# trzy/FasterRCNN

Measured on AMD Instinct MI355X. Metric: images/sec (600x1000) Faster-RCNN VGG-16 inference, higher is better.
Workload: dtype f32 (float32 tensors and accumulation; 15 GEMM layers in the f32x3 split-operand emulation = two fp16 terms per block-scaled operand, three fp16 MFMAs per product; 0 in f32x6 = three bf16 terms, six bf16 MFMAs; the other 2 on exact-f32 MFMA; strict exact-f32 everywhere: config.strict_f32_images_per_

## Files before the change

### fasterrcnn_amd/csrc/wino_x3f.hip

```cpp
#include "x3t.h"

namespace frcnn {

typedef _Float16 xf_f16x8 __attribute__((ext_vector_type(8)));

static constexpr int XF_TC = 16;
static constexpr int XF_HC = 2 * XF_TC + 2;
static constexpr int XF_PS = 20;
static constexpr int X3_HR = 10;


struct XfGeom { int tbx, tby, ncb, tw, th, xg; unsigned m_tbx, m_tby, m_ncb; int ntb; unsigned m_ntb; int g8; int n_items; };
__device__ __forceinline__ int xd_div(int n, int d, unsigned m) { return d == 1 ? n : (int)__umulhi((unsigned)n, m); }

typedef float xd_f32x2 __attribute__((ext_vector_type(2)));
typedef _Float16 xd_f16x2 __attribute__((ext_vector_type(2)));

static constexpr int XD_HP = XF_HC / 2;
static constexpr int XD_NDMA = 7;
static constexpr int XD_HBUF_BYTES = XD_NDMA * 256 * 16;
static constexpr int XD_HBUF_FLOATS = XD_HBUF_BYTES / 4;
typedef __attribute__((address_space(3))) void* xd_lds_ptr;
static constexpr int XD_MS = 68;
static constexpr int XD_M_BYTES = 16 * 32 * XD_MS * 4;
static constexpr int XD_SC_OFFSET = XD_M_BYTES;
static constexpr int XD_CM_OFFSET = XD_SC_OFFSET + 16 * 64 * 4 + 64 * 4;
static constexpr size_t XD_LDS_BYTES = XD_CM_OFFSET + 512 * 4;

template <int N> struct XdInt { static constexpr int value = N; };
#ifndef XD_ABLATE
#define XD_ABLATE 0
#endif

__device__ __forceinline__ float xd_rowmax16(float v)
{
    v = fmaxf(v, __builtin_bit_cast(float, __builtin_amdgcn_update_dpp(0, __builtin_bit_cast(int, v), 0x128, 0xf, 0xf, false)));
    v = fmaxf(v, __builtin_bit_cast(float, __builtin_amdgcn_update_dpp(0, __builtin_bit_cast(int, v), 0x124, 0xf, 0xf, false)));
    v = fmaxf(v, __builtin_bit_cast(float, __builtin_amdgcn_update_dpp(0, __builtin_bit_cast(int, v), 0x122, 0xf, 0xf, false)));
    v = fmaxf(v, __builtin_bit_cast(float, __builtin_amdgcn_update_dpp(0, __builtin_bit_cast(int, v), 0x121, 0xf, 0xf, false)));
    return v;
}

__device__ __forceinline__ f32x4 xd_sub4(f32x4 a, f32x4 b)
{
    xd_f32x2 a0 = {a[0], a[1]}, a1 = {a[2], a[3]}, b0 = {b[0], b[1]}, b1 = {b[2], b[3]}, r0, r1;
    asm("v_pk_add_f32 %0, %1, %2 neg_lo:[0,1] neg_hi:[0,1]" : "=v"(r0) : "v"(a0), "v"(b0));
    asm("v_pk_add_f32 %0, %1, %2 neg_lo:[0,1] neg_hi:[0,1]" : "=v"(r1) : "v"(a1), "v"(b1));
    return f32x4{r0[0], r0[1], r1[0], r1[1]};
}

__device__ __forceinline__ void xd_slot_tile(int s, int& ty, int& tx)
{
    ty = (int)((0xF00F0FF0u >> s) & 1u);
    tx = s - 4 * ((s + 4) >> 3);
}

__device__ __forceinline__ void xd_lds_barrier()
{
    asm volatile("s_waitcnt lgkmcnt(0)\n\ts_barrier" ::: "memory");
}


__device__ __forceinline__ bool xd_block_to_tile(const XfGeom& gm, int b, int& cb, int& bx, int& by, int& map)
{
    if (gm.xg == 2) {
        const int xcd = b & 7, s = b >> 3;
        if (gm.ncb >= 8) {
            const int k = xd_div(s, gm.ntb, gm.m_ntb);
            cb = xcd + 8 * k;
            b = s - k * gm.ntb;
        } else {
            const int g = gm.g8, sub = xd_div(xcd, gm.ncb, gm.m_ncb);
            cb = xcd - sub * gm.ncb;
            b = s * g + sub;
            if (b >= gm.ntb) return false;
        }
    } else if (gm.xg) {
        const int xcd = b & 7, q = b >> 3, qq = xd_div(q, gm.ncb, gm.m_ncb);
        cb = q - qq * gm.ncb;
        b = qq * 8 + xcd;
    } else {
        const int qq = xd_div(b, gm.ncb, gm.m_ncb);
        cb = b - qq * gm.ncb;
        b = qq;
    }
    const int b1 = xd_div(b, gm.tbx, gm.m_tbx);
    bx = b - b1 * gm.tbx;
    map = xd_div(b1, gm.tby, gm.m_tby);
    by = b1 - map * gm.tby;
    return true;
}


typedef unsigned xp_u32x4_t __attribute__((ext_vector_type(4)));


__device__ __forceinline__ float xd_rowmax16_scatter16(const float (&v)[16])
{
    float n0, n1, n2, n3, n4, n5, n6, n7;
    asm volatile("s_nop 1\n\t"
        "v_max_f32_dpp %0, %8, %8 row_ror:8 row_mask:0xf bank_mask:0x3\n\tv_max_f32_dpp %1, %9, %9 row_ror:8 row_mask:0xf bank_mask:0x3\n\t"
        "v_max_f32_dpp %2, %10, %10 row_ror:8 row_mask:0xf bank_mask:0x3\n\tv_max_f32_dpp %3, %11, %11 row_ror:8 row_mask:0xf bank_mask:0x3\n\t"
        "v_max_f32_dpp %4, %12, %12 row_ror:8 row_mask:0xf bank_mask:0x3\n\tv_max_f32_dpp %5, %13, %13 row_ror:8 row_mask:0xf bank_mask:0x3\n\t"
        "v_max_f32_dpp %6, %14, %14 row_ror:8 row_mask:0xf bank_mask:0x3\n\tv_max_f32_dpp %7, %15, %15 row_ror:8 row_mask:0xf bank_mask:0x3\n\t"
        "v_max_f32_dpp %0, %16, %16 row_ror:8 row_mask:0xf bank_mask:0xc\n\tv_max_f32_dpp %1, %17, %17 row_ror:8 row_mask:0xf bank_mask:0xc\n\t"
        "v_max_f32_dpp %2, %18, %18 row_ror:8 row_mask:0xf bank_mask:0xc\n\tv_max_f32_dpp %3, %19, %19 row_ror:8 row_mask:0xf bank_mask:0xc\n\t"
        "v_max_f32_dpp %4, %20, %20 row_ror:8 row_mask:0xf bank_mask:0xc\n\tv_max_f32_dpp %5, %21, %21 row_ror:8 row_mask:0xf bank_mask:0xc\n\t"
        "v_max_f32_dpp %6, %22, %22 row_ror:8 row_mask:0xf bank_mask:0xc\n\tv_max_f32_dpp %7, %23, %23 row_ror:8 row_mask:0xf bank_mask:0xc"
        : "=&v"(n0), "=&v"(n1), "=&v"(n2), "=&v"(n3), "=&v"(n4), "=&v"(n5), "=&v"(n6), "=&v"(n7)
        : "v"(v[0]), "v"(v[1]), "v"(v[2]), "v"(v[3]), "v"(v[4]), "v"(v[5]), "v"(v[6]), "v"(v[7]),
          "v"(v[8]), "v"(v[9]), "v"(v[10]), "v"(v[11]), "v"(v[12]), "v"(v[13]), "v"(v[14]), "v"(v[15]));
    float m0, m1, m2, m3;
    asm volatile(
        "v_max_f32_dpp %0, %4, %4 row_ror:12 row_mask:0xf bank_mask:0x5\n\tv_max_f32_dpp %1, %5, %5 row_ror:12 row_mask:0xf bank_mask:0x5\n\t"
        "v_max_f32_dpp %2, %6, %6 row_ror:12 row_mask:0xf bank_mask:0x5\n\tv_max_f32_dpp %3, %7, %7 row_ror:12 row_mask:0xf bank_mask:0x5\n\t"
        "v_max_f32_dpp %0, %8, %8 row_ror:4 row_mask:0xf bank_mask:0xa\n\tv_max_f32_dpp %1, %9, %9 row_ror:4 row_mask:0xf bank_mask:0xa\n\t"
        "v_max_f32_dpp %2, %10, %10 row_ror:4 row_mask:0xf bank_mask:0xa\n\tv_max_f32_dpp %3, %11, %11 row_ror:4 row_mask:0xf bank_mask:0xa\n\t"
        "v_max_f32_dpp %0, %0, %0 quad_perm:[2,3,0,1] row_mask:0xf bank_mask:0xf\n\tv_max_f32_dpp %1, %1, %1 quad_perm:[2,3,0,1] row_mask:0xf bank_mask:0xf\n\t"
        "v_max_f32_dpp %2, %2, %2 quad_perm:[2,3,0,1] row_mask:0xf bank_mask:0xf\n\tv_max_f32_dpp %3, %3, %3 quad_perm:[2,3,0,1] row_mask:0xf bank_mask:0xf\n\t"
        "v_max_f32_dpp %0, %0, %0 quad_perm:[1,0,3,2] row_mask:0xf bank_mask:0xf\n\tv_max_f32_dpp %1, %1, %1 quad_perm:[1,0,3,2] row_mask:0xf bank_mask:0xf\n\t"
        "v_max_f32_dpp %2, %2, %2 quad_perm:[1,0,3,2] row_mask:0xf bank_mask:0xf\n\tv_max_f32_dpp %3, %3, %3 quad_perm:[1,0,3,2] row_mask:0xf bank_mask:0xf\n\t"
        "s_nop 1"
        : "=&v"(m0), "=&v"(m1), "=&v"(m2), "=&v"(m3)
        : "v"(n0), "v"(n1), "v"(n2), "v"(n3), "v"(n4), "v"(n5), "v"(n6), "v"(n7));
    const int q = (int)(threadIdx.x & 3);
    return q == 0 ? m0 : q == 1 ? m1 : q == 2 ? m2 : m3;
}
__device__ __forceinline__ float xd_rowmax16_scatter4(const float (&v)[4])
{
    float n0, n1, m;
    asm volatile("s_nop 1\n\t"
        "v_max_f32_dpp %0, %3, %3 row_ror:8 row_mask:0xf bank_mask:0x3\n\tv_max_f32_dpp %1, %4, %4 row_ror:8 row_mask:0xf bank_mask:0x3\n\t"
        "v_max_f32_dpp %0, %5, %5 row_ror:8 row_mask:0xf bank_mask:0xc\n\tv_max_f32_dpp %1, %6, %6 row_ror:8 row_mask:0xf bank_mask:0xc\n\t"
        "s_nop 1\n\t"
        "v_max_f32_dpp %2, %0, %0 row_ror:12 row_mask:0xf bank_mask:0x5\n\tv_max_f32_dpp %2, %1, %1 row_ror:4 row_mask:0xf bank_mask:0xa\n\t"
        "s_nop 1\n\t"
        "v_max_f32_dpp %2, %2, %2 quad_perm:[2,3,0,1] row_mask:0xf bank_mask:0xf\n\t"
        "s_nop 1\n\t"
        "v_max_f32_dpp %2, %2, %2 quad_perm:[1,0,3,2] row_mask:0xf bank_mask:0xf\n\t"
        "s_nop 1"
        : "=&v"(n0), "=&v"(n1), "=&v"(m)
        : "v"(v[0]), "v"(v[1]), "v"(v[2]), "v"(v[3]));
    return m;
}

#ifndef XD_EARLY_HALO
#define XD_EARLY_HALO 1
#endif
static constexpr int XD_FIRST = 1, XD_EARLY = XD_EARLY_HALO ? 2 : 0, XD_LAST = 4;

template <bool POOL, bool TWO>
__global__ __launch_bounds__(256, 1)
void wino_x3d_kernel(const float* __restrict__ x_maps, const float* __restrict__ cmax_maps, const unsigned char* __restrict__ ublob,
                     const float* __restrict__ bias, float* __restrict__ y_maps, int H, int W, int Cin, int Cout, int u_rbt, int relu,
                     XfGeom gm, float* __restrict__ cmax_out_maps)
{
#ifdef XD_CLOCKS
    const unsigned long long xd_t_in = __builtin_amdgcn_s_memrealtime();
#endif
    extern __shared__ __attribute__((aligned(16))) unsigned char smem_xf[];
    float* const hbuf0 = reinterpret_cast<float*>(smem_xf);

#ifndef XD_PERSIST
    const int tid = threadIdx.x, lane = tid & 63;
    const int wave = __builtin_amdgcn_readfirstlane(tid >> 6);
#endif
    const int K16 = Cin >> 4;

#ifdef XD_PERSIST
    for (int item = blockIdx.x; item < gm.n_items; item += gridDim.x) {
    int tid_l = threadIdx.x;
#if XD_PERSIST >= 2
    asm volatile("" : "+v"(tid_l));
#endif
    const int tid = tid_l, lane = tid & 63;
    const int wave = __builtin_amdgcn_readfirstlane((int)threadIdx.x >> 6);
#else
    {
    const int item = blockIdx.x;
#endif
    int cb, bx, by, map;
    if (!xd_block_to_tile(gm, item, cb, bx, by, map)) {
#ifdef XD_PERSIST
        continue;
#else
        return;
#endif
    }
    const float* __restrict__ const x = x_maps + (size_t)map * H * W * Cin;
    const float* __restrict__ const cmax = cmax_maps + (size_t)map * H * W;
    float* __restrict__ const y = y_maps + (size_t)map * (POOL ? (size_t)(H >> 1) * (W >> 1) : (size_t)H * W) * Cout;
    float* __restrict__ const cmax_out = cmax_out_maps ? cmax_out_maps + (size_t)map * (POOL ? (size_t)(H >> 1) * (W >> 1) : (size_t)H * W) : nullptr;

    const __amdgpu_buffer_rsrc_t xrs = __builtin_amdgcn_make_buffer_rsrc(const_cast<float*>(x), 0, H * W * Cin * (int)sizeof(float), 0x00020000);
    const __amdgpu_buffer_rsrc_t mrs = __builtin_amdgcn_make_buffer_rsrc(const_cast<float*>(cmax), 0, H * W * (int)sizeof(float), 0x00020000);

    const int tl = lane & 31, kh = lane >> 5;
    int tyl, txl;
    xd_slot_tile(tl, tyl, txl);
    float mult[2], vinv[2];

    const int hy0 = 8 * by - 1, hx0 = 2 * XF_TC * bx - 1;
    const int wave_u = __builtin_amdgcn_readfirstlane(wave);
    int h_src[XD_NDMA];
    auto halo_source = [&](auto IT) {
        constexpr int it = decltype(IT)::value;
        const unsigned P = (unsigned)((it * 4 + wave) * 64 + lane);
        const unsigned slot = __umul24(P, 52429u) >> 18, part = P - 5u * slot;
        const unsigned hr = __umul24(slot, 1928u) >> 16, rem = slot - (unsigned)XF_HC * hr;
        const unsigned par = rem >= (unsigned)XD_HP ? 1u : 0u, hc = 2u * (rem - par * (unsigned)XD_HP) + par;
        const int gy = hy0 + (int)hr, gx = hx0 + (int)hc;
        bool inb = (part < 4u) & ((unsigned)gy < (unsigned)H) & ((unsigned)gx < (unsigned)W);
        if (it == XD_NDMA - 1) inb &= hr < (unsigned)X3_HR;
        const unsigned off = (__umul24((unsigned)gy, (unsigned)W) + (unsigned)gx) * (unsigned)(Cin * 4) + 16u * part;
        h_src[it] = inb ? (int)off : (int)0xFFFFFFF0u;
    };
    __amdgpu_buffer_rsrc_t xrs_ring = xrs;
    auto dma_halo = [&](float* hb, int chunk_off, auto IT0, auto IT1, const __amdgpu_buffer_rsrc_t& rs) {
        if (XD_ABLATE & 8) return;
#pragma unroll
        for (int it = decltype(IT0)::value; it < decltype(IT1)::value; ++it)
            __builtin_amdgcn_raw_ptr_buffer_load_lds(rs, (xd_lds_ptr)(reinterpret_cast<unsigned char*>(hb) + (it * 4 + wave_u) * 1024), 16, h_src[it],
                                                     chunk_off, 0, 0);
    };

    xf_f16x8 U[2][4][2][2];
    const __amdgpu_buffer_rsrc_t urs = __builtin_amdgcn_make_buffer_rsrc(const_cast<unsigned char*>(ublob), 0, 16 * K16 * u_rbt * HX_RB, 0x00020000);
    const int chunk_stride = u_rbt * HX_RB;
    int ubase[4];
#pragma unroll
    for (int j = 0; j < 4; ++j) ubase[j] = ((4 * wave + j) * K16 * u_rbt + 2 * cb) * HX_RB;
    const int lane16 = lane * 16;
    auto load_u = [&](int chunk, auto SET, auto J) {
        constexpr int set = decltype(SET)::value, j = decltype(J)::value;
        const int so = ubase[j] + chunk * chunk_stride;
#pragma unroll
        for (int ct = 0; ct < 2; ++ct)
#pragma unroll
            for (int t = 0; t < 2; ++t)
                U[set][j][ct][t] = __builtin_bit_cast(xf_f16x8, __builtin_amdgcn_raw_buffer_load_b128(urs, lane16, so + ct * HX_RB + t * HX_PIECE, 0));
    };

    f32x16 acc[2][4][2];

    const int a1 = wave == 0 ? 0 : (wave == 2 ? 2 : 1);
    const int a2 = wave == 0 ? 2 : (wave == 2 ? 1 : (wave == 1 ? 2 : 3));
    const float rsgn = wave != 1 ? -1.0f : 1.0f;
    const int d_lane = (4 * tyl * XD_HP + txl) * XF_PS + 8 * kh;
    float r[4][8];
    f32x4 du0, du1, dw0, dw1;
    auto read_d = [&](const float* hb, int h, int bb) {
        const float* p1 = hb + d_lane + (((4 * h + a1) * 2 + (bb & 1)) * XD_HP + (bb >> 1)) * XF_PS;
        const float* p2 = hb + d_lane + (((4 * h + a2) * 2 + (bb & 1)) * XD_HP + (bb >> 1)) * XF_PS;
        du0 = *reinterpret_cast<const f32x4*>(p1); du1 = *reinterpret_cast<const f32x4*>(p1 + 4);
        dw0 = *reinterpret_cast<const f32x4*>(p2); dw1 = *reinterpret_cast<const f32x4*>(p2 + 4);
    };
    auto read_d_lo = [&](const float* hb, int h, int bb) {
        const float* p1 = hb + d_lane + (((4 * h + a1) * 2 + (bb & 1)) * XD_HP + (bb >> 1)) * XF_PS;
        const float* p2 = hb + d_lane + (((4 * h + a2) * 2 + (bb & 1)) * XD_HP + (bb >> 1)) * XF_PS;
        du0 = *reinterpret_cast<const f32x4*>(p1);
        dw0 = *reinterpret_cast<const f32x4*>(p2);
    };
    auto read_d_hi = [&](const float* hb, int h, int bb) {
        const float* p1 = hb + d_lane + (((4 * h + a1) * 2 + (bb & 1)) * XD_HP + (bb >> 1)) * XF_PS;
        const float* p2 = hb + d_lane + (((4 * h + a2) * 2 + (bb & 1)) * XD_HP + (bb >> 1)) * XF_PS;
        du1 = *reinterpret_cast<const f32x4*>(p1 + 4);
        dw1 = *reinterpret_cast<const f32x4*>(p2 + 4);
    };
    auto make_r = [&](int bb, int half, int hs) {
        const bool scaled = bb == 1 || bb == 2;
#pragma unroll
        for (int e = 0; e < 4; ++e) {
            float v = half == 0 ? __builtin_fmaf(dw0[e], rsgn, du0[e]) : __builtin_fmaf(dw1[e], rsgn, du1[e]);
            if (scaled) asm volatile("v_mul_f32 %0, %1, %2" : "=v"(v) : "v"(v), "v"(mult[hs]));
            r[bb][4 * half + e] = v;
        }
    };
    unsigned vhi[2][4], vlo[2][4];
    float tt[4];
    auto v_adds = [&](int h, int j, int e2) {
#pragma unroll
        for (int q = 0; q < 4; ++q) {
            const int e = 2 * e2 + q;
            tt[q] = j == 0 ? __builtin_fmaf(r[0][e], mult[h], -r[2][e]) : j == 1 ? r[1][e] + r[2][e] : j == 2 ? r[2][e] - r[1][e]
                                                                                                   : __builtin_fmaf(r[3][e], -mult[h], r[1][e]);
        }
    };
    auto v_hi = [&](int slot, int e2) {
        unsigned ha, hb;
        asm("v_cvt_pk_f16_f32 %0, %1, %2" : "=v"(ha) : "v"(tt[0]), "v"(tt[1]));
        asm("v_cvt_pk_f16_f32 %0, %1, %2" : "=v"(hb) : "v"(tt[2]), "v"(tt[3]));
        vhi[slot][e2] = ha;
        vhi[slot][e2 + 1] = hb;
    };
    auto v_lo = [&](int slot, int e2) {
        unsigned la, lb;
        asm("v_fma_mixlo_f16 %0, %2, 1.0, -%6 op_sel:[0,0,0] op_sel_hi:[0,0,1]\n\tv_fma_mixlo_f16 %1, %4, 1.0, -%7 op_sel:[0,0,0] op_sel_hi:[0,0,1]\n\t"
            "v_fma_mixhi_f16 %0, %3, 1.0, -%6 op_sel:[0,0,1] op_sel_hi:[0,0,1]\n\tv_fma_mixhi_f16 %1, %5, 1.0, -%7 op_sel:[0,0,1] op_sel_hi:[0,0,1]"
            : "=&v"(la), "=&v"(lb) : "v"(tt[0]), "v"(tt[1]), "v"(tt[2]), "v"(tt[3]), "v"(vhi[slot][e2]), "v"(vhi[slot][e2 + 1]));
        vlo[slot][e2] = la;
        vlo[slot][e2 + 1] = lb;
    };
    auto frag = [&](const unsigned (&q)[4]) { return __builtin_bit_cast(xf_f16x8, uint4{q[0], q[1], q[2], q[3]}); };
#define XD_MFMA(SET, H_, J_, CT, UT, VV) \
    do { if (!(XD_ABLATE & 16)) acc[H_][J_][CT] = __builtin_amdgcn_mfma_f32_32x32x16_f16(U[SET][J_][CT][UT], VV, acc[H_][J_][CT], 0, 0, 0); } while (0)
#define XD_MFMA0(SET, H_, J_, CT, UT, VV) \
    do { if (first) acc[H_][J_][CT] = __builtin_amdgcn_mfma_f32_32x32x16_f16(U[SET][J_][CT][UT], VV, xd_zero16, 0, 0, 0); else XD_MFMA(SET, H_, J_, CT, UT, VV); } while (0)
#define XD_FENCE() __builtin_amdgcn_sched_barrier(0)
#define XD_IF(BIT, STMT) do { if (!(XD_ABLATE & (BIT))) { STMT; } } while (0)

#ifdef XD_STEPS
    unsigned long long xd_step_acc[8] = {0, 0, 0, 0, 0, 0, 0, 0}, xd_step_last = 0;
#endif
    auto step = [&](int ucb, int hso, int hso_next, float* hcur, float* hnxt, float* hthird_, auto PAR, auto S, auto FLAGS) {
        constexpr int par = decltype(PAR)::value, s = decltype(S)::value;
#ifdef XD_STEPS
        {
            const unsigned long long now = __builtin_readcyclecounter();
            if (xd_step_last != 0) xd_step_acc[(s + 7) & 7] += now - xd_step_last;
            xd_step_last = now;
        }
#endif
        constexpr bool first = (decltype(FLAGS)::value & XD_FIRST) != 0, early = (decltype(FLAGS)::value & XD_EARLY) != 0,
                       last = (decltype(FLAGS)::value & XD_LAST) != 0;
        const f32x16 xd_zero16 = {};
        constexpr int h = s >> 2, j = s & 3, slot = s & 1, nslot = slot ^ 1;
        constexpr int nh = s == 3 ? 1 : s == 7 ? 0 : h, nj = (j + 1) & 3;
        constexpr int rb = j == 0 ? 0 : j == 1 ? 2 : j == 2 ? 1 : 3;
        constexpr int prb = j == 0 ? 3 : j == 1 ? 0 : j == 2 ? 2 : 1;
        constexpr int rh = h ^ 1;
        constexpr int prh = j == 0 ? h : rh;
        constexpr bool col = !(last && h == 1), pcol = !(last && s >= 5), form = !(last && s == 7);
        const float* rsrc = h == 0 ? hcur : hnxt;
        const xf_f16x8 vh = frag(vhi[slot]), vl = frag(vlo[slot]);
        XD_MFMA0(par, h, j, 0, 1, vh);
        if (col) XD_IF(2, read_d_lo(rsrc, rh, rb));
        if (form) XD_IF(1, v_adds(nh, nj, 0));
        XD_FENCE();
        XD_MFMA0(par, h, j, 1, 1, vh);
        if (form) XD_IF(1, v_hi(nslot, 0));
        if (pcol) XD_IF(2, make_r(prb, 1, prh));
        XD_FENCE();
        XD_MFMA(par, h, j, 0, 0, vh);
        if (form) XD_IF(1, v_lo(nslot, 0));
        if (col) XD_IF(2, read_d_hi(rsrc, rh, rb));
        if (s == 4 && !last) dma_halo(hcur, hso, XdInt<0>{}, XdInt<4>{}, xrs_ring);
        if (early && !last && !(XD_EARLY_HALO == 2 && TWO) && s == 0) dma_halo(XD_EARLY_HALO == 2 ? hthird_ : hnxt, hso_next + (XD_EARLY_HALO == 2 ? 64 : 0), XdInt<0>{}, XdInt<4>{}, xrs);
        if (early && !last && !(XD_EARLY_HALO == 2 && TWO) && s == 1) dma_halo(XD_EARLY_HALO == 2 ? hthird_ : hnxt, hso_next + (XD_EARLY_HALO == 2 ? 64 : 0), XdInt<4>{}, XdInt<XD_NDMA>{}, xrs);
        XD_FENCE();
        XD_MFMA(par, h, j, 1, 0, vh);
        if (form) XD_IF(1, v_adds(nh, nj, 2));
        if (form) XD_IF(1, v_hi(nslot, 2));
        XD_FENCE();
        XD_MFMA(par, h, j, 0, 0, vl);
        if (form) XD_IF(1, v_lo(nslot, 2));
        if (!last && !(XD_ABLATE & 4)) {
            const int so = ubase[s >> 1] + ucb;
            U[par ^ 1][s >> 1][s & 1][0] = __builtin_bit_cast(xf_f16x8, __builtin_amdgcn_raw_buffer_load_b128(urs, lane16 + (s & 1) * HX_RB, so, 0));
            U[par ^ 1][s >> 1][s & 1][1] = __builtin_bit_cast(xf_f16x8, __builtin_amdgcn_raw_buffer_load_b128(urs, lane16 + (s & 1) * HX_RB + HX_PIECE, so, 0));
        }
        XD_FENCE();
        XD_MFMA(par, h, j, 1, 0, vl);
        if (col) XD_IF(2, make_r(rb, 0, rh));
        if (s == 3) {
            if (early) asm volatile("s_waitcnt vmcnt(%0)" ::"n"(XD_EARLY_HALO == 2 ? (last ? 0 : TWO ? 8 : 15) : (last ? 0 : 6)) : "memory");
            else asm volatile("s_waitcnt vmcnt(15)" ::: "memory");
            xd_lds_barrier();
        }
        if (s == 5 && !last) dma_halo(hcur, hso, XdInt<4>{}, XdInt<XD_NDMA>{}, xrs_ring);
        XD_FENCE();
    };
    float *hcur = hbuf0, *hnxt = hbuf0 + XD_HBUF_FLOATS, *hthird = hbuf0 + 2 * XD_HBUF_FLOATS;
    auto chunk = [&](int c, auto PAR, auto FLAGS) {
        const int ucb = (c + 1) * chunk_stride, hso = (c + 3 < K16 ? c + 3 : K16 - 1) * 64, hson = (c + 1) * 64;
        xrs_ring = __builtin_amdgcn_make_buffer_rsrc(const_cast<float*>(x), 0, c + 3 < K16 ? H * W * Cin * (int)sizeof(float) : 0, 0x00020000);
        step(ucb, hso, hson, hcur, hnxt, hthird, PAR, XdInt<0>{}, FLAGS); step(ucb, hso, hson, hcur, hnxt, hthird, PAR, XdInt<1>{}, FLAGS);
        step(ucb, hso, hson, hcur, hnxt, hthird, PAR, XdInt<2>{}, FLAGS); step(ucb, hso, hson, hcur, hnxt, hthird, PAR, XdInt<3>{}, FLAGS);
        step(ucb, hso, hson, hcur, hnxt, hthird, PAR, XdInt<4>{}, FLAGS); step(ucb, hso, hson, hcur, hnxt, hthird, PAR, XdInt<5>{}, FLAGS);
        step(ucb, hso, hson, hcur, hnxt, hthird, PAR, XdInt<6>{}, FLAGS); step(ucb, hso, hson, hcur, hnxt, hthird, PAR, XdInt<7>{}, FLAGS);
        float* const t = hcur; hcur = hnxt; hnxt = hthird; hthird = t;
    };

    float* const sc_lds = reinterpret_cast<float*>(smem_xf + XD_SC_OFFSET);
    const float* const uinv0 = reinterpret_cast<const float*>(ublob + (size_t)16 * K16 * u_rbt * HX_RB) + (size_t)(tid >> 4) * (u_rbt * 32) + 64 * cb + (tid & 15) * 4;
    int cm_src[2];
#pragma unroll
    for (int q = 0; q < 2; ++q) {
        const unsigned P = (unsigned)(tid + 256 * q);
        const unsigned hr = __umul24(P, 1928u) >> 16, hc = P - (unsigned)XF_HC * hr;
        const int gy = hy0 + (int)hr, gx = hx0 + (int)hc;
        const bool inb = (hr < (unsigned)X3_HR) & ((unsigned)gy < (unsigned)H) & ((unsigned)gx < (unsigned)W);
        cm_src[q] = inb ? (int)((__umul24((unsigned)gy, (unsigned)W) + (unsigned)gx) * 4u) : (int)0xFFFFFFF0u;
    }
    XD_FENCE();
    auto load_u1 = [&](auto J, auto CT, auto T) {
        constexpr int j = decltype(J)::value, ct = decltype(CT)::value, tt_ = decltype(T)::value;
        U[0][j][ct][tt_] = __builtin_bit_cast(xf_f16x8, __builtin_amdgcn_raw_buffer_load_b128(urs, lane16, ubase[j] + ct * HX_RB + tt_ * HX_PIECE, 0));
    };
    __builtin_amdgcn_raw_ptr_buffer_load_lds(mrs, (xd_lds_ptr)(smem_xf + XD_CM_OFFSET + (0 * 4 + wave_u) * 256), 4, cm_src[0], 0, 0, 0);
    halo_source(XdInt<0>{}); XD_FENCE();
    __builtin_amdgcn_raw_ptr_buffer_load_lds(mrs, (xd_lds_ptr)(smem_xf + XD_CM_OFFSET + (1 * 4 + wave_u) * 256), 4, cm_src[1], 0, 0, 0);
    halo_source(XdInt<1>{}); XD_FENCE();
    if (!(XD_ABLATE & 32)) load_u1(XdInt<0>{}, XdInt<0>{}, XdInt<0>{});
    halo_source(XdInt<2>{}); XD_FENCE();
    if (!(XD_ABLATE & 32)) load_u1(XdInt<0>{}, XdInt<0>{}, XdInt<1>{});
    halo_source(XdInt<3>{}); XD_FENCE();
    if (!(XD_ABLATE & 32)) load_u1(XdInt<0>{}, XdInt<1>{}, XdInt<0>{});
    halo_source(XdInt<4>{}); XD_FENCE();
    if (!(XD_ABLATE & 32)) load_u1(XdInt<0>{}, XdInt<1>{}, XdInt<1>{});
    halo_source(XdInt<5>{}); halo_source(XdInt<6>{}); XD_FENCE();
    if (!(XD_ABLATE & 32)) dma_halo(hcur, 0, XdInt<0>{}, XdInt<XD_NDMA>{}, xrs);
    __builtin_amdgcn_global_load_lds(uinv0, (xd_lds_ptr)(smem_xf + XD_SC_OFFSET + wave_u * 1024), 16, 0, 0);
    const xd_lds_ptr bias_lds = (xd_lds_ptr)(smem_xf + XD_SC_OFFSET + 4096);
    if (wave_u == 0 && lane < 16) __builtin_amdgcn_global_load_lds(bias + 64 * cb + 4 * lane, bias_lds, 16, 0, 0);
    XD_FENCE();
    if (!(XD_ABLATE & 32)) { load_u(0, XdInt<0>{}, XdInt<1>{}); load_u(0, XdInt<0>{}, XdInt<2>{}); load_u(0, XdInt<0>{}, XdInt<3>{}); }
    XD_FENCE();
    if (XD_EARLY_HALO != 1 && !(XD_ABLATE & 32)) {
        dma_halo(hnxt, 64, XdInt<0>{}, XdInt<XD_NDMA>{}, xrs);
        if (XD_EARLY_HALO == 0 && !TWO) dma_halo(hthird, 128, XdInt<0>{}, XdInt<XD_NDMA>{}, xrs);
    }
    XD_FENCE();
#ifdef XD_CLOCKS
    const unsigned long long xd_t_issued = __builtin_amdgcn_s_memrealtime();
#endif
    asm volatile("s_waitcnt vmcnt(%0)" ::"n"((XD_ABLATE & 32) ? 0 : 12 + (XD_EARLY_HALO == 1 ? 0 : XD_EARLY_HALO == 2 ? XD_NDMA : (TWO ? 1 : 2) * XD_NDMA)) : "memory");
    xd_lds_barrier();
    {
        const float* cm = reinterpret_cast<const float*>(smem_xf + XD_CM_OFFSET) + (2 * tyl) * XF_HC + 2 * txl;
#pragma unroll
        for (int h = 0; h < 2; ++h) {
            float dmax = 0.f;
#pragma unroll
            for (int a = 0; a < 4; ++a) {
                const xd_f32x2 u = *reinterpret_cast<const xd_f32x2*>(cm + (4 * h + a) * XF_HC);
                const xd_f32x2 v = *reinterpret_cast<const xd_f32x2*>(cm + (4 * h + a) * XF_HC + 2);
                dmax = fmaxf(fmaxf(dmax, fmaxf(u[0], u[1])), fmaxf(v[0], v[1]));
            }
            hx_row_scale(4.0f * dmax, mult[h], vinv[h]);
        }
    }
#ifdef XD_CLOCKS
    const unsigned long long xd_t_landed = __builtin_amdgcn_s_memrealtime();
#endif
#pragma unroll
    for (int bb = 0; bb < 4; ++bb) { read_d(hcur, 0, bb); make_r(bb, 0, 0); make_r(bb, 1, 0); }
    v_adds(0, 0, 0); v_hi(0, 0); v_lo(0, 0);
    v_adds(0, 0, 2); v_hi(0, 2); v_lo(0, 2);
#ifdef XD_CLOCKS
    const unsigned long long xd_t_loop = __builtin_amdgcn_s_memrealtime(), xd_c_loop = __builtin_readcyclecounter();
#endif
    chunk(0, XdInt<0>{}, XdInt<XD_FIRST | XD_EARLY>{});
#ifdef XD_CHUNK_CLOCKS
    const unsigned long long xd_c_k0 = __builtin_readcyclecounter();
    unsigned long long xd_c_k1 = xd_c_k0, xd_c_kl = xd_c_k0, xd_c_kl2 = xd_c_k0;
#endif
    if constexpr (TWO) {
        int one = 1;
        asm volatile("" : "+s"(one));
        for (int rep = 0; rep < one; ++rep) chunk(1, XdInt<1>{}, XdInt<(XD_EARLY_HALO == 1 ? XD_EARLY : 0) | XD_LAST>{});
    } else {
        chunk(1, XdInt<1>{}, XdInt<(XD_EARLY_HALO == 1 ? XD_EARLY : 0)>{});
#ifdef XD_CHUNK_CLOCKS
        xd_c_k1 = __builtin_readcyclecounter();
#endif
        for (int c = 2; c < K16 - 2; c += 2) {
            chunk(c, XdInt<0>{}, XdInt<0>{});
            chunk(c + 1, XdInt<1>{}, XdInt<0>{});
        }
#ifdef XD_CHUNK_CLOCKS
        xd_c_kl2 = __builtin_readcyclecounter();
#endif
        chunk(K16 - 2, XdInt<0>{}, XdInt<0>{});
#ifdef XD_CHUNK_CLOCKS
        xd_c_kl = __builtin_readcyclecounter();
#endif
        int one = 1;
        asm volatile("" : "+s"(one));
        for (int rep = 0; rep < one; ++rep) chunk(K16 - 1, XdInt<1>{}, XdInt<XD_LAST>{});
    }
#undef XD_MFMA
#undef XD_MFMA0
#undef XD_FENCE
#undef XD_IF
#ifdef XD_CLOCKS
    const unsigned long long xd_t_done = __builtin_amdgcn_s_memrealtime(), xd_c_done = __builtin_readcyclecounter();
#endif
    asm volatile("s_waitcnt vmcnt(0)" ::: "memory");
    __syncthreads();
#ifdef XD_CLOCKS
    const unsigned long long xd_t_e0 = __builtin_amdgcn_s_memrealtime();
#endif

    float* const ybuf = reinterpret_cast<float*>(smem_xf);
#pragma unroll
    for (int ct = 0; ct < 2; ++ct)
#pragma unroll
        for (int g = 0; g < 4; ++g) {
            const int co = 32 * ct + 8 * g + 4 * kh;
            f32x4 sb[4];
#pragma unroll
            for (int j = 0; j < 4; ++j) sb[j] = *reinterpret_cast<const f32x4*>(sc_lds + (4 * wave + j) * 64 + co);
#pragma unroll
            for (int h = 0; h < 2; ++h) {
                f32x4 a[4];
#pragma unroll
                for (int j = 0; j < 4; ++j) a[j] = f32x4{acc[h][j][ct][4 * g], acc[h][j][ct][4 * g + 1], acc[h][j][ct][4 * g + 2], acc[h][j][ct][4 * g + 3]};
                const f32x4 vi = {vinv[h], vinv[h], vinv[h], vinv[h]};
                const f32x4 y0 = __builtin_elementwise_fma(a[2], sb[2], __builtin_elementwise_fma(a[1], sb[1], a[0] * sb[0])) * vi;
                const f32x4 y1 = __builtin_elementwise_fma(a[3], -sb[3], __builtin_elementwise_fma(a[2], -sb[2], a[1] * sb[1])) * vi;
                float* dst = ybuf + ((((h * 4 + wave) * 2) * 32 + tl) * XD_MS) + co;
                *reinterpret_cast<f32x4*>(dst) = y0;
                *reinterpret_cast<f32x4*>(dst + 32 * XD_MS) = y1;
            }
        }
    __syncthreads();
#ifdef XD_CLOCKS
    const unsigned long long xd_t_e1 = __builtin_amdgcn_s_memrealtime();
#endif
    const int Ho = H >> 1, Wo = W >> 1;
    const float lowb = relu ? 0.f : -__builtin_inff();
    auto xmax = [](float a, float b) { float r; asm("v_max_f32 %0, %1, %2" : "=v"(r) : "v"(a), "v"(b)); return r; };
    const __amdgpu_buffer_rsrc_t yrs = __builtin_amdgcn_make_buffer_rsrc(y, 0, (POOL ? Ho * Wo : H * W) * Cout * (int)sizeof(float), 0x00020000);
    float pmv[POOL ? 4 : 16];
#pragma unroll
    for (int it = 0; it < 4; ++it) {
        const int item = tid + 256 * it;
        const int t = item >> 4, k = (item & 15) * 4;
        const int h = t >> 5, tt_ = t & 31;
        int sty, stx;
        xd_slot_tile(tt_, sty, stx);
        const int oty = 4 * by + 2 * h + sty, otx = XF_TC * bx + stx;
        const int kg = 64 * cb + k;
        const float* yp = ybuf + ((h * 4) * 2 * 32 + tt_) * XD_MS + k;
        f32x4 Y[4][2];
#pragma unroll
        for (int i = 0; i < 4; ++i)
#pragma unroll
            for (int bb = 0; bb < 2; ++bb) Y[i][bb] = *reinterpret_cast<const f32x4*>(yp + (i * 2 + bb) * (32 * XD_MS));
        const f32x4 bv = *reinterpret_cast<const f32x4*>(sc_lds + 1024 + k);
        f32x4 o[2][2];
#pragma unroll
        for (int bb = 0; bb < 2; ++bb) {
            o[0][bb] = ((Y[0][bb] + Y[1][bb]) + Y[2][bb]) + bv;
            o[1][bb] = xd_sub4(xd_sub4(Y[1][bb], Y[2][bb]), Y[3][bb]) + bv;
        }
        if constexpr (POOL) {
            f32x4 mx;
#pragma unroll
            for (int e = 0; e < 4; ++e) {
                float m3;
                asm("v_max3_f32 %0, %1, %2, %3" : "=v"(m3) : "v"(o[0][0][e]), "v"(o[0][1][e]), "v"(o[1][0][e]));
                asm("v_max3_f32 %0, %1, %2, %3" : "=v"(mx[e]) : "v"(m3), "v"(o[1][1][e]), "v"(lowb));
            }
            const bool live = (oty < Ho) & (otx < Wo);
            const int off = live ? ((oty * Wo + otx) * Cout + kg) * 4 : (int)0xFFFFFFF0u;
            __builtin_amdgcn_raw_buffer_store_b128(__builtin_bit_cast(xp_u32x4_t, mx), yrs, off, 0, 0);
            { float m3; asm("v_max3_f32 %0, %1, %2, %3" : "=v"(m3) : "v"(mx[0]), "v"(mx[1]), "v"(mx[2])); pmv[it] = xmax(m3, mx[3]); }
        } else {
            const int base = ((2 * oty * W + 2 * otx) * Cout + kg) * 4;
#pragma unroll
            for (int a = 0; a < 2; ++a) {
#pragma unroll
                for (int bb = 0; bb < 2; ++bb) {
                    const bool ok = (2 * oty + a < H) & (2 * otx + bb < W);
#pragma unroll
                    for (int e = 0; e < 4; ++e) o[a][bb][e] = xmax(o[a][bb][e], lowb);
                    const int off = ok ? base + (a * W + bb) * Cout * 4 : (int)0xFFFFFFF0u;
                    __builtin_amdgcn_raw_buffer_store_b128(__builtin_bit_cast(xp_u32x4_t, o[a][bb]), yrs, off, 0, 0);
                    { float m3; asm("v_max3_f32 %0, %1, %2, %3" : "=v"(m3) : "v"(o[a][bb][0]), "v"(o[a][bb][1]), "v"(o[a][bb][2])); pmv[it * 4 + a * 2 + bb] = xmax(m3, o[a][bb][3]); }
                }
            }
        }
    }
    if (cmax_out) {
        const int li = tid & 15, itl = li >> 2;
        const int t = (tid >> 4) + 16 * itl, h = t >> 5, tt_ = t & 31;
        int sty, stx;
        xd_slot_tile(tt_, sty, stx);
        const int oty = 4 * by + 2 * h + sty, otx = XF_TC * bx + stx;
        if constexpr (POOL) {
            const float pm = xd_rowmax16_scatter4(reinterpret_cast<const float (&)[4]>(pmv));
            const bool live = oty < gm.th && otx < gm.tw && oty < Ho && otx < Wo;
            if (live && (li & 3) == 0) atomicMax(reinterpret_cast<unsigned*>(cmax_out + (size_t)oty * Wo + otx), __float_as_uint(pm));
        } else {
            const float pm = xd_rowmax16_scatter16(reinterpret_cast<const float (&)[16]>(pmv));
            const int yy = 2 * oty + ((li >> 1) & 1), xx = 2 * otx + (li & 1);
            const bool ok = oty < gm.th && otx < gm.tw && yy < H && xx < W;
            if (ok) atomicMax(reinterpret_cast<unsigned*>(cmax_out + (size_t)yy * W + xx), __float_as_uint(pm));
        }
    }
#ifdef XD_PERSIST
    __syncthreads();
#endif
#ifdef XD_CLOCKS
    if (tid == 0) {
        const unsigned long long t_out = __builtin_amdgcn_s_memrealtime();
        float* rec = y_maps + (POOL ? (size_t)(H >> 1) * (W >> 1) : (size_t)H * W) * Cout + (size_t)blockIdx.x * 16;
        rec[0] = (float)(xd_t_loop - xd_t_in); rec[1] = (float)(xd_t_done - xd_t_loop); rec[2] = (float)(t_out - xd_t_done);
        rec[3] = (float)(xd_c_done - xd_c_loop); rec[4] = (float)(xd_t_in & 0xFFFFFF); rec[5] = (float)(t_out & 0xFFFFFF);
        rec[6] = (float)K16; rec[7] = 1.0f;
        rec[8] = (float)(xd_t_issued - xd_t_in); rec[9] = (float)(xd_t_landed - xd_t_issued); rec[10] = (float)(xd_t_loop - xd_t_landed);
        rec[11] = (float)(xd_t_e0 - xd_t_done); rec[12] = (float)(xd_t_e1 - xd_t_e0); rec[13] = (float)(t_out - xd_t_e1);
#ifdef XD_CHUNK_CLOCKS
        rec[8] = (float)(xd_c_k0 - xd_c_loop); rec[9] = (float)(xd_c_k1 - xd_c_k0); rec[10] = (float)(xd_c_kl2 - xd_c_k1);
        rec[11] = (float)(xd_c_kl - xd_c_kl2); rec[12] = (float)(xd_c_done - xd_c_kl);
#endif
#ifdef XD_STEPS
        for (int q = 0; q < 8; ++q) rec[8 + q] = (float)xd_step_acc[q];
#endif
    }
#endif
    }
}

size_t conv3x3_winograd_x3_fused_workspace_bytes(int N, int H, int W) { return (size_t)N * H * W * sizeof(float); }

int launch_conv3x3_winograd_x3_fused(const float* x, const void* ublob, const float* b, float* y, int N, int H, int W, int cin, int cout,
                                     unsigned flags, void* ws, size_t ws_bytes, hipStream_t s, const float* cmax_ready, float* cmax_out)
{
    if (N < 1 || H < 1 || W < 1 || cin < 32 || cin % 32 != 0 || cout < 64 || cout % 64 != 0) return FRCNN_EUNSUPPORTED;
    if ((size_t)H * W * cin >= ((size_t)1 << 29) || (size_t)H * W * cout >= ((size_t)1 << 29)) return FRCNN_EUNSUPPORTED;
    if ((flags & FRCNN_POOL2) && (H < 2 || W < 2)) return FRCNN_EINVAL;
    if (!cmax_ready && (!ws || ws_bytes < conv3x3_winograd_x3_fused_workspace_bytes(N, H, W))) return FRCNN_EINVAL;
    if (cmax_out && !(flags & FRCNN_RELU)) return FRCNN_EINVAL;
    const float* cmax = cmax_ready;
    if (!cmax) {
        int rc = launch_pixel_absmax(x, static_cast<float*>(ws), (long long)N * H * W, cin, s);
        if (rc) return rc;
        cmax = static_cast<const float*>(ws);
    }
    XfGeom gm;
    gm.tw = cdiv(W, 2); gm.th = cdiv(H, 2);
    gm.tbx = cdiv(gm.tw, XF_TC); gm.tby = cdiv(gm.th, 4);
    gm.ncb = cout / 64;
    const long long total = (long long)gm.tbx * gm.tby * gm.ncb * N;
    if (total > 0x7fffffffLL) return FRCNN_EINVAL;
    gm.xg = ((long long)gm.tbx * gm.tby * N) % 8 == 0 ? 1 : 0;
    gm.ntb = gm.tbx * gm.tby * N;
    long long grid_blocks = total;
#ifndef XD_NO_FILTER_RESIDENT
    if (cin >= 256 && (gm.ncb % 8 == 0 || 8 % gm.ncb == 0)) {
        gm.xg = 2;
        if (gm.ncb < 8) grid_blocks = 8LL * cdiv(gm.ntb, 8 / gm.ncb);
    }
#endif
    auto magic = [](int d) { return d == 1 ? 0u : (unsigned)((0x100000000ull + (unsigned)d - 1) / (unsigned)d); };
    gm.m_tbx = magic(gm.tbx); gm.m_tby = magic(gm.tby); gm.m_ncb = magic(gm.ncb); gm.m_ntb = magic(gm.ntb);
    gm.g8 = gm.ncb < 8 ? 8 / gm.ncb : 1;
    gm.n_items = (int)grid_blocks;
#ifdef XD_PERSIST
    if (grid_blocks > 256) grid_blocks = 256;
#endif
    if (total * std::max(std::max(gm.ncb, gm.ntb), std::max(gm.tbx, gm.tby)) >= 0x100000000ll) return FRCNN_EUNSUPPORTED;
    const int u_rbt = cdiv(cout, gemm_x6t_col_tile(cout)) * gemm_x6t_col_tile(cout) / 32;
    if ((size_t)16 * (cin / 16) * u_rbt * HX_RB >= ((size_t)1 << 31)) return FRCNN_EUNSUPPORTED;
    const int relu = (flags & FRCNN_RELU) ? 1 : 0;
    const unsigned char* ub = static_cast<const unsigned char*>(ublob);
#define XD_LAUNCH(P_, T_)                                                                                                                    \
    do {                                                                                                                                    \
        auto kern = wino_x3d_kernel<P_, T_>;                                                                                                \
        FRCNN_MAX_LDS_ONCE(kern, XD_LDS_BYTES);                                                                                             \
        hipLaunchKernelGGL(kern, dim3((unsigned)grid_blocks), dim3(256), XD_LDS_BYTES, s, x, cmax, ub, b, y, H, W, cin, cout, u_rbt, relu, gm, cmax_out); \
    } while (0)
    if (flags & FRCNN_POOL2) { if (cin == 32) XD_LAUNCH(true, true); else XD_LAUNCH(true, false); }
    else                     { if (cin == 32) XD_LAUNCH(false, true); else XD_LAUNCH(false, false); }
#undef XD_LAUNCH
    return check_launch();
}

}
```

Measured before the change: 930.0.

## Add half-tile Winograd body for bottom-edge blocks to skip dead rows

Moves the fused Winograd x3 conv kernel body into a templated device function with a HALF variant. It runs for blocks whose second tile row lies past the image height. The HALF path loads fewer halo DMA pieces and skips the second half of the channel-max loads, MFMAs, epilogue and store iterations, using its own 4-step chunk schedule with different wait counts. This targets wasted work on partial bottom tiles, at the cost of a second code instantiation and a distinct synchronization schedule that must be kept correct.

```diff
diff --git a/fasterrcnn_amd/csrc/wino_x3f.hip b/fasterrcnn_amd/csrc/wino_x3f.hip
--- a/fasterrcnn_amd/csrc/wino_x3f.hip
+++ b/fasterrcnn_amd/csrc/wino_x3f.hip
@@ -18,6 +18,7 @@
 
 static constexpr int XD_HP = XF_HC / 2;
 static constexpr int XD_NDMA = 7;
+static constexpr int XD_NDMA_HALF = 4;
 static constexpr int XD_HBUF_BYTES = XD_NDMA * 256 * 16;
 static constexpr int XD_HBUF_FLOATS = XD_HBUF_BYTES / 4;
 typedef __attribute__((address_space(3))) void* xd_lds_ptr;
@@ -149,44 +150,27 @@
 #endif
 static constexpr int XD_FIRST = 1, XD_EARLY = XD_EARLY_HALO ? 2 : 0, XD_LAST = 4;
 
-template <bool POOL, bool TWO>
-__global__ __launch_bounds__(256, 1)
-void wino_x3d_kernel(const float* __restrict__ x_maps, const float* __restrict__ cmax_maps, const unsigned char* __restrict__ ublob,
-                     const float* __restrict__ bias, float* __restrict__ y_maps, int H, int W, int Cin, int Cout, int u_rbt, int relu,
-                     XfGeom gm, float* __restrict__ cmax_out_maps)
-{
-#ifdef XD_CLOCKS
-    const unsigned long long xd_t_in = __builtin_amdgcn_s_memrealtime();
-#endif
+template <bool POOL, bool TWO, bool HALF>
+__device__ __forceinline__
+void xd_body(const float* __restrict__ x_maps, const float* __restrict__ cmax_maps, const unsigned char* __restrict__ ublob,
+             const float* __restrict__ bias, float* __restrict__ y_maps, int H, int W, int Cin, int Cout, int u_rbt, int relu,
+             const XfGeom& gm, float* __restrict__ cmax_out_maps, const int cb, const int bx, const int by, const int map
+#ifdef XD_CLOCKS
+             , const unsigned long long xd_t_in
+#endif
+             )
+{
     extern __shared__ __attribute__((aligned(16))) unsigned char smem_xf[];
     float* const hbuf0 = reinterpret_cast<float*>(smem_xf);
 
-#ifndef XD_PERSIST
-    const int tid = threadIdx.x, lane = tid & 63;
-    const int wave = __builtin_amdgcn_readfirstlane(tid >> 6);
-#endif
-    const int K16 = Cin >> 4;
-
-#ifdef XD_PERSIST
-    for (int item = blockIdx.x; item < gm.n_items; item += gridDim.x) {
     int tid_l = threadIdx.x;
-#if XD_PERSIST >= 2
+#if defined(XD_PERSIST) && XD_PERSIST >= 2
     asm volatile("" : "+v"(tid_l));
 #endif
     const int tid = tid_l, lane = tid & 63;
     const int wave = __builtin_amdgcn_readfirstlane((int)threadIdx.x >> 6);
-#else
+    const int K16 = Cin >> 4;
     {
-    const int item = blockIdx.x;
-#endif
-    int cb, bx, by, map;
-    if (!xd_block_to_tile(gm, item, cb, bx, by, map)) {
-#ifdef XD_PERSIST
-        continue;
-#else
-        return;
-#endif
-    }
     const float* __restrict__ const x = x_maps + (size_t)map * H * W * Cin;
     const float* __restrict__ const cmax = cmax_maps + (size_t)map * H * W;
     float* __restrict__ const y = y_maps + (size_t)map * (POOL ? (size_t)(H >> 1) * (W >> 1) : (size_t)H * W) * Cout;
@@ -380,6 +364,61 @@
         step(ucb, hso, hson, hcur, hnxt, hthird, PAR, XdInt<6>{}, FLAGS); step(ucb, hso, hson, hcur, hnxt, hthird, PAR, XdInt<7>{}, FLAGS);
         float* const t = hcur; hcur = hnxt; hnxt = hthird; hthird = t;
     };
+    auto hstep = [&](int ucb, int hso, float* hfree, float* hread, auto PAR, auto S, auto FLAGS) {
+        constexpr int par = decltype(PAR)::value, s = decltype(S)::value;
+        constexpr bool first = (decltype(FLAGS)::value & XD_FIRST) != 0, last = (decltype(FLAGS)::value & XD_LAST) != 0;
+        const f32x16 xd_zero16 = {};
+        constexpr int j = s, slot = s & 1, nslot = slot ^ 1, nj = (j + 1) & 3;
+        constexpr int rb = j == 0 ? 0 : j == 1 ? 2 : j == 2 ? 1 : 3;
+        constexpr int prb = j == 0 ? 3 : j == 1 ? 0 : j == 2 ? 2 : 1;
+        constexpr bool col = !last, pcol = !(last && s >= 1), form = !(last && s == 3);
+        const xf_f16x8 vh = frag(vhi[slot]), vl = frag(vlo[slot]);
+        XD_MFMA0(par, 0, j, 0, 1, vh);
+        if (col) XD_IF(2, read_d_lo(hread, 0, rb));
+        if (form) XD_IF(1, v_adds(0, nj, 0));
+        XD_FENCE();
+        XD_MFMA0(par, 0, j, 1, 1, vh);
+        if (form) XD_IF(1, v_hi(nslot, 0));
+        if (pcol) XD_IF(2, make_r(prb, 1, 0));
+        XD_FENCE();
+        XD_MFMA(par, 0, j, 0, 0, vh);
+        if (form) XD_IF(1, v_lo(nslot, 0));
+        if (col) XD_IF(2, read_d_hi(hread, 0, rb));
+        if (s == 0 && !last) dma_halo(hfree, hso, XdInt<0>{}, XdInt<2>{}, xrs_ring);
+        if (s == 1 && !last) dma_halo(hfree, hso, XdInt<2>{}, XdInt<XD_NDMA_HALF>{}, xrs_ring);
+        XD_FENCE();
+        XD_MFMA(par, 0, j, 1, 0, vh);
+        if (form) XD_IF(1, v_adds(0, nj, 2));
+        if (form) XD_IF(1, v_hi(nslot, 2));
+        XD_FENCE();
+        XD_MFMA(par, 0, j, 0, 0, vl);
+        if (form) XD_IF(1, v_lo(nslot, 2));
+        if (!last) {
+            const int so = ubase[j] + ucb;
+            U[par ^ 1][j][0][0] = __builtin_bit_cast(xf_f16x8, __builtin_amdgcn_raw_buffer_load_b128(urs, lane16, so, 0));
+            U[par ^ 1][j][0][1] = __builtin_bit_cast(xf_f16x8, __builtin_amdgcn_raw_buffer_load_b128(urs, lane16 + HX_PIECE, so, 0));
+        }
+        XD_FENCE();
+        XD_MFMA(par, 0, j, 1, 0, vl);
+        if (!last) {
+            const int so = ubase[j] + ucb;
+            U[par ^ 1][j][1][0] = __builtin_bit_cast(xf_f16x8, __builtin_amdgcn_raw_buffer_load_b128(urs, lane16 + HX_RB, so, 0));
+            U[par ^ 1][j][1][1] = __builtin_bit_cast(xf_f16x8, __builtin_amdgcn_raw_buffer_load_b128(urs, lane16 + HX_RB + HX_PIECE, so, 0));
+        }
+        if (col) XD_IF(2, make_r(rb, 0, 0));
+        if (s == 3 && !last) {
+            asm volatile("s_waitcnt vmcnt(%0)" ::"n"(XD_NDMA_HALF + 16) : "memory");
+            xd_lds_barrier();
+        }
+        XD_FENCE();
+    };
+    auto hchunk = [&](int c, auto PAR, auto FLAGS) {
+        const int ucb = (c + 1) * chunk_stride, hso = (c + 3 < K16 ? c + 3 : K16 - 1) * 64;
+        xrs_ring = __builtin_amdgcn_make_buffer_rsrc(const_cast<float*>(x), 0, c + 3 < K16 ? H * W * Cin * (int)sizeof(float) : 0, 0x00020000);
+        hstep(ucb, hso, hcur, hnxt, PAR, XdInt<0>{}, FLAGS); hstep(ucb, hso, hcur, hnxt, PAR, XdInt<1>{}, FLAGS);
+        hstep(ucb, hso, hcur, hnxt, PAR, XdInt<2>{}, FLAGS); hstep(ucb, hso, hcur, hnxt, PAR, XdInt<3>{}, FLAGS);
+        float* const t = hcur; hcur = hnxt; hnxt = hthird; hthird = t;
+    };
 
     float* const sc_lds = reinterpret_cast<float*>(smem_xf + XD_SC_OFFSET);
     const float* const uinv0 = reinterpret_cast<const float*>(ublob + (size_t)16 * K16 * u_rbt * HX_RB) + (size_t)(tid >> 4) * (u_rbt * 32) + 64 * cb + (tid & 15) * 4;
@@ -399,37 +438,41 @@
     };
     __builtin_amdgcn_raw_ptr_buffer_load_lds(mrs, (xd_lds_ptr)(smem_xf + XD_CM_OFFSET + (0 * 4 + wave_u) * 256), 4, cm_src[0], 0, 0, 0);
     halo_source(XdInt<0>{}); XD_FENCE();
-    __builtin_amdgcn_raw_ptr_buffer_load_lds(mrs, (xd_lds_ptr)(smem_xf + XD_CM_OFFSET + (1 * 4 + wave_u) * 256), 4, cm_src[1], 0, 0, 0);
+    if (!HALF) __builtin_amdgcn_raw_ptr_buffer_load_lds(mrs, (xd_lds_ptr)(smem_xf + XD_CM_OFFSET + (1 * 4 + wave_u) * 256), 4, cm_src[1], 0, 0, 0);
     halo_source(XdInt<1>{}); XD_FENCE();
     if (!(XD_ABLATE & 32)) load_u1(XdInt<0>{}, XdInt<0>{}, XdInt<0>{});
     halo_source(XdInt<2>{}); XD_FENCE();
     if (!(XD_ABLATE & 32)) load_u1(XdInt<0>{}, XdInt<0>{}, XdInt<1>{});
     halo_source(XdInt<3>{}); XD_FENCE();
     if (!(XD_ABLATE & 32)) load_u1(XdInt<0>{}, XdInt<1>{}, XdInt<0>{});
-    halo_source(XdInt<4>{}); XD_FENCE();
+    if (!HALF) halo_source(XdInt<4>{});
+    XD_FENCE();
     if (!(XD_ABLATE & 32)) load_u1(XdInt<0>{}, XdInt<1>{}, XdInt<1>{});
-    halo_source(XdInt<5>{}); halo_source(XdInt<6>{}); XD_FENCE();
-    if (!(XD_ABLATE & 32)) dma_halo(hcur, 0, XdInt<0>{}, XdInt<XD_NDMA>{}, xrs);
+    if (!HALF) { halo_source(XdInt<5>{}); halo_source(XdInt<6>{}); }
+    XD_FENCE();
+    constexpr int NDMA = HALF ? XD_NDMA_HALF : XD_NDMA;
+    if (!(XD_ABLATE & 32)) dma_halo(hcur, 0, XdInt<0>{}, XdInt<NDMA>{}, xrs);
     __builtin_amdgcn_global_load_lds(uinv0, (xd_lds_ptr)(smem_xf + XD_SC_OFFSET + wave_u * 1024), 16, 0, 0);
     const xd_lds_ptr bias_lds = (xd_lds_ptr)(smem_xf + XD_SC_OFFSET + 4096);
     if (wave_u == 0 && lane < 16) __builtin_amdgcn_global_load_lds(bias + 64 * cb + 4 * lane, bias_lds, 16, 0, 0);
     XD_FENCE();
     if (!(XD_ABLATE & 32)) { load_u(0, XdInt<0>{}, XdInt<1>{}); load_u(0, XdInt<0>{}, XdInt<2>{}); load_u(0, XdInt<0>{}, XdInt<3>{}); }
     XD_FENCE();
-    if (XD_EARLY_HALO != 1 && !(XD_ABLATE & 32)) {
-        dma_halo(hnxt, 64, XdInt<0>{}, XdInt<XD_NDMA>{}, xrs);
-        if (XD_EARLY_HALO == 0 && !TWO) dma_halo(hthird, 128, XdInt<0>{}, XdInt<XD_NDMA>{}, xrs);
+    constexpr int early_mode = HALF ? 0 : XD_EARLY_HALO;
+    if (early_mode != 1 && !(XD_ABLATE & 32)) {
+        dma_halo(hnxt, 64, XdInt<0>{}, XdInt<NDMA>{}, xrs);
+        if (early_mode == 0 && !TWO) dma_halo(hthird, 128, XdInt<0>{}, XdInt<NDMA>{}, xrs);
     }
     XD_FENCE();
 #ifdef XD_CLOCKS
     const unsigned long long xd_t_issued = __builtin_amdgcn_s_memrealtime();
 #endif
-    asm volatile("s_waitcnt vmcnt(%0)" ::"n"((XD_ABLATE & 32) ? 0 : 12 + (XD_EARLY_HALO == 1 ? 0 : XD_EARLY_HALO == 2 ? XD_NDMA : (TWO ? 1 : 2) * XD_NDMA)) : "memory");
+    asm volatile("s_waitcnt vmcnt(%0)" ::"n"((XD_ABLATE & 32) ? 0 : 12 + (early_mode == 1 ? 0 : early_mode == 2 ? NDMA : (TWO ? 1 : 2) * NDMA)) : "memory");
     xd_lds_barrier();
     {
         const float* cm = reinterpret_cast<const float*>(smem_xf + XD_CM_OFFSET) + (2 * tyl) * XF_HC + 2 * txl;
 #pragma unroll
-        for (int h = 0; h < 2; ++h) {
+        for (int h = 0; h < (HALF ? 1 : 2); ++h) {
             float dmax = 0.f;
 #pragma unroll
             for (int a = 0; a < 4; ++a) {
@@ -450,7 +493,15 @@
 #ifdef XD_CLOCKS
     const unsigned long long xd_t_loop = __builtin_amdgcn_s_memrealtime(), xd_c_loop = __builtin_readcyclecounter();
 #endif
-    chunk(0, XdInt<0>{}, XdInt<XD_FIRST | XD_EARLY>{});
+    if constexpr (HALF) {
+        asm volatile("s_waitcnt vmcnt(%0)" ::"n"(TWO ? 0 : XD_NDMA_HALF) : "memory");
+        xd_lds_barrier();
+    }
+    auto run_chunk = [&](int c, auto PAR, auto FLAGS) {
+        if constexpr (HALF) hchunk(c, PAR, XdInt<(decltype(FLAGS)::value & ~XD_EARLY)>{});
+        else chunk(c, PAR, FLAGS);
+    };
+    run_chunk(0, XdInt<0>{}, XdInt<XD_FIRST | XD_EARLY>{});
 #ifdef XD_CHUNK_CLOCKS
     const unsigned long long xd_c_k0 = __builtin_readcyclecounter();
     unsigned long long xd_c_k1 = xd_c_k0, xd_c_kl = xd_c_k0, xd_c_kl2 = xd_c_k0;
@@ -458,26 +509,26 @@
     if constexpr (TWO) {
         int one = 1;
         asm volatile("" : "+s"(one));
-        for (int rep = 0; rep < one; ++rep) chunk(1, XdInt<1>{}, XdInt<(XD_EARLY_HALO == 1 ? XD_EARLY : 0) | XD_LAST>{});
+        for (int rep = 0; rep < one; ++rep) run_chunk(1, XdInt<1>{}, XdInt<(XD_EARLY_HALO == 1 ? XD_EARLY : 0) | XD_LAST>{});
     } else {
-        chunk(1, XdInt<1>{}, XdInt<(XD_EARLY_HALO == 1 ? XD_EARLY : 0)>{});
+        run_chunk(1, XdInt<1>{}, XdInt<(XD_EARLY_HALO == 1 ? XD_EARLY : 0)>{});
 #ifdef XD_CHUNK_CLOCKS
         xd_c_k1 = __builtin_readcyclecounter();
 #endif
         for (int c = 2; c < K16 - 2; c += 2) {
-            chunk(c, XdInt<0>{}, XdInt<0>{});
-            chunk(c + 1, XdInt<1>{}, XdInt<0>{});
+            run_chunk(c, XdInt<0>{}, XdInt<0>{});
+            run_chunk(c + 1, XdInt<1>{}, XdInt<0>{});
         }
 #ifdef XD_CHUNK_CLOCKS
         xd_c_kl2 = __builtin_readcyclecounter();
 #endif
-        chunk(K16 - 2, XdInt<0>{}, XdInt<0>{});
+        run_chunk(K16 - 2, XdInt<0>{}, XdInt<0>{});
 #ifdef XD_CHUNK_CLOCKS
         xd_c_kl = __builtin_readcyclecounter();
 #endif
         int one = 1;
         asm volatile("" : "+s"(one));
-        for (int rep = 0; rep < one; ++rep) chunk(K16 - 1, XdInt<1>{}, XdInt<XD_LAST>{});
+        for (int rep = 0; rep < one; ++rep) run_chunk(K16 - 1, XdInt<1>{}, XdInt<XD_LAST>{});
     }
 #undef XD_MFMA
 #undef XD_MFMA0
@@ -502,7 +553,7 @@
 #pragma unroll
             for (int j = 0; j < 4; ++j) sb[j] = *reinterpret_cast<const f32x4*>(sc_lds + (4 * wave + j) * 64 + co);
 #pragma unroll
-            for (int h = 0; h < 2; ++h) {
+            for (int h = 0; h < (HALF ? 1 : 2); ++h) {
                 f32x4 a[4];
 #pragma unroll
                 for (int j = 0; j < 4; ++j) a[j] = f32x4{acc[h][j][ct][4 * g], acc[h][j][ct][4 * g + 1], acc[h][j][ct][4 * g + 2], acc[h][j][ct][4 * g + 3]};
@@ -523,8 +574,12 @@
     auto xmax = [](float a, float b) { float r; asm("v_max_f32 %0, %1, %2" : "=v"(r) : "v"(a), "v"(b)); return r; };
     const __amdgpu_buffer_rsrc_t yrs = __builtin_amdgcn_make_buffer_rsrc(y, 0, (POOL ? Ho * Wo : H * W) * Cout * (int)sizeof(float), 0x00020000);
     float pmv[POOL ? 4 : 16];
-#pragma unroll
-    for (int it = 0; it < 4; ++it) {
+    if constexpr (HALF) {
+#pragma unroll
+        for (int q = (POOL ? 2 : 8); q < (POOL ? 4 : 16); ++q) pmv[q] = 0.f;
+    }
+#pragma unroll
+    for (int it = 0; it < (HALF ? 2 : 4); ++it) {
         const int item = tid + 256 * it;
         const int t = item >> 4, k = (item & 15) * 4;
         const int h = t >> 5, tt_ = t & 31;
@@ -614,6 +669,33 @@
     }
 }
 
+template <bool POOL, bool TWO>
+__global__ __launch_bounds__(256, 1)
+void wino_x3d_kernel(const float* __restrict__ x_maps, const float* __restrict__ cmax_maps, const unsigned char* __restrict__ ublob,
+                     const float* __restrict__ bias, float* __restrict__ y_maps, int H, int W, int Cin, int Cout, int u_rbt, int relu,
+                     XfGeom gm, float* __restrict__ cmax_out_maps)
+{
+#ifdef XD_CLOCKS
+    const unsigned long long xd_t_in = __builtin_amdgcn_s_memrealtime();
+#define XD_T_IN , xd_t_in
+#else
+#define XD_T_IN
+#endif
+#ifdef XD_PERSIST
+    for (int item = blockIdx.x; item < gm.n_items; item += gridDim.x) {
+#else
+    {
+    const int item = blockIdx.x;
+#endif
+    int cb, bx, by, map;
+    if (xd_block_to_tile(gm, item, cb, bx, by, map)) {
+        if (4 * by + 2 >= gm.th) xd_body<POOL, TWO, true>(x_maps, cmax_maps, ublob, bias, y_maps, H, W, Cin, Cout, u_rbt, relu, gm, cmax_out_maps, cb, bx, by, map XD_T_IN);
+        else xd_body<POOL, TWO, false>(x_maps, cmax_maps, ublob, bias, y_maps, H, W, Cin, Cout, u_rbt, relu, gm, cmax_out_maps, cb, bx, by, map XD_T_IN);
+    }
+    }
+#undef XD_T_IN
+}
+
 size_t conv3x3_winograd_x3_fused_workspace_bytes(int N, int H, int W) { return (size_t)N * H * W * sizeof(float); }
 
 int launch_conv3x3_winograd_x3_fused(const float* x, const void* ublob, const float* b, float* y, int N, int H, int W, int cin, int cout,
```

Result: no change. 936.3, median of 6 (+0.7%).
